# QizhiPei/FABind

Measured on AMD Instinct MI355X. Metric: complexes/sec fwd+bwd (1500p/40l nodes), full IaBNet on the whole graph (pocket model + 4-layer complex model + distance-map head on all nodes / pairs) with the pocket-cls + pocket-centre + coord + distmap + distmap-by-coords + distill losses (BASELINE configs[2] read literally), higher is better.
Workload: dtype bf16

## Files before the change

### fabind_amd/_lib.py

```python
import ctypes
import os

import torch

from . import config as _cfg

_HERE = os.path.dirname(os.path.abspath(__file__))
LIB_PATH = _cfg.knob("FABIND_LIB") or os.path.join(_HERE, "libfabind_hip.so")

ABI_VERSION = 19
DT_F32, DT_BF16 = 0, 1
ACT_NONE, ACT_SILU, ACT_RELU, ACT_SIGMOID, ACT_STORED_DERIV = 0, 1, 2, 3, 4
GEMM_FAM_NT_F32, GEMM_FAM_NT_F32_BF16, GEMM_FAM_NT_BF16, GEMM_FAM_GLDS, GEMM_FAM_PIPE, GEMM_FAM_X3, GEMM_FAM_X3_PRO, GEMM_FAM_PERSIST = range(8)

LNR_8S16, LNR_8S32, LNR_V8_1, LNR_V8_2, LNR_V8_3, LNR_V8_4, LNR_S2, LNR_S8, LNR_S16, LNR_S32, LNR_COUNT = range(11)
LNB_8S16, LNB_8S32, LNB_V8_1, LNB_V8_2, LNB_V8_3, LNB_S2, LNB_S8, LNB_S16, LNB_S20, LNB_S32, LNB_COUNT = range(11)
RST_BF16_1, RST_BF16_2, RST_BF16_4, RST_GENERIC, RST_COUNT = range(5)
ELF_WAVE1, ELF_WAVE1_TAIL, ELF_WAVE2_TAIL, ELF_CHUNK, ELF_COUNT = range(5)
ELB_NPL1, ELB_NPL2, ELB_NPL3, ELB_COUNT = range(4)

_vp, _i, _f, _l = ctypes.c_void_p, ctypes.c_int, ctypes.c_float, ctypes.c_long


class GemmArgs(ctypes.Structure):
# ... 125 lines not shown
    "fabind_rowdot_bwd": [_vp, _i, _vp, _i, _vp, _i, _i, _i, _vp, _vp, _vp, _i, _vp],
    "fabind_edge_geom_bwd": [_vp, _vp, _vp, _vp, _vp, _vp, _vp, _vp, _vp, _vp, _i, _i, _i, _vp, _vp, _vp, _vp],
    "fabind_gcl_pre_bwd": [_vp, _i, _i, _vp, _vp, _i, _vp, _vp, _vp, _i, _vp],
    "fabind_gather_dact": [_vp, _i, _vp, _vp, _i, _i, _vp, _i, _i, _i, _vp],
    "fabind_coord_update_bwd": [_vp, _vp, _vp, _i, _i, _f, _vp, _vp, _vp, _vp],
    "fabind_cross_attn_bwd": [_vp, _i, _vp, _i, _vp, _i, _i, _i, _vp, _i, _i, _i, _f, _vp, _vp, _vp, _vp, _vp, _vp, _vp,
                              _vp, _vp, _vp],
    "fabind_pair_bias_cat": [_vp, _i, _vp, _i, _i, _i, _vp, _i, _vp, _i, _vp, _vp, _i, _vp, _i, _vp, _vp],
    "fabind_batched_transpose_pad": [_vp, _i, _vp, _i, _i, _i, _i, _vp, _vp],
    "fabind_node_chain_fwd": [_vp, _i, _vp, _i, _vp, _vp, _vp, _vp, _vp, _vp, _i, _i, _vp, _i, _vp, _i, _vp, _i, _i, _i, _vp],
    "fabind_node_chain_x3_fwd": [_vp, _i, _vp, _i, _vp, _vp, _vp, _vp, _vp, _vp, _vp, _vp, _vp, _vp, _i, _i, _vp, _i, _vp, _i, _vp, _i, _vp, _i, _vp, _i,
                                 _i, _i, _vp],
    "fabind_rows_hadamard_bwd": [_vp, _i, _i, _vp, _i, _i, _vp, _vp, _vp, _i, _vp, _i, _vp],
    "fabind_pair_hadamard_bwd_grid": [_vp, _i, _i, _vp, _i, _i, _vp, _vp, _vp, _vp, _i, _vp, _i, _vp],
    "fabind_pair_hadamard_bwd_rows": [_vp, _i, _i, _vp, _i, _i, _vp, _i, _i, _vp, _vp, _vp, _vp, _i, _vp, _i, _vp, _i, _vp],
    "fabind_pair_hadamard_bwd": [_vp, _i, _i, _vp, _vp, _i, _i, _vp, _vp, _i, _i, _vp, _vp, _i, _vp, _vp, _i, _vp, _vp, _i,
                                 _vp],
    "fabind_inter_attn_bwd": [_vp, _i, _vp, _i, _i, _vp, _vp, _vp, _vp, _vp, _vp, _vp, _vp, _vp, _vp, _vp, _vp, _f, _i,
                              _vp, _vp, _vp, _vp, _vp, _vp, _vp, _vp, _vp, _vp, _i, _vp],
    "fabind_inter_attn_bwd_rows": [_vp, _i, _vp, _i, _i, _vp, _vp, _vp, _vp, _vp, _vp, _vp, _vp, _vp, _vp, _vp, _vp, _f, _i,
                                   _vp, _vp, _vp, _vp, _vp, _vp, _vp, _vp, _vp, _vp, _i, _vp, _i, _i, _vp],
    "fabind_las_step_bwd": [_vp, _vp, _vp, _vp, _vp, _vp, _vp, _vp, _i, _i, _f, _f, _vp, _vp, _vp],
    "fabind_pair_bias_bwd": [_vp, _i, _vp, _i, _i, _vp, _vp, _i, _i, _i, _vp, _vp, _vp, _vp, _vp],
    "fabind_pair_bias_btcat": [_vp, _i, _vp, _vp, _vp, _i, _i, _i, _vp, _i, _i, _vp],
    "fabind_pair_bias_finish": [_vp, _vp, _i, _i, _vp, _vp, _i, _vp, _vp, _l, _vp],
    "fabind_pack_frag_multi": [_vp, _vp, _i, _vp],
    "fabind_lower_bound": [_vp, _i, _vp, _i, _vp, _vp],
    "fabind_pocket_center_fwd": [_vp, _vp, _vp, _vp, _i, _i, _f, _i, _vp, _vp, _vp],
    "fabind_pocket_center_bwd": [_vp, _vp, _vp, _vp, _i, _i, _f, _vp, _vp, _vp, _vp, _vp],
    "fabind_pair_dist_fwd": [_vp, _i, _i, _vp, _vp, _f, _f, _f, _vp, _vp],
    "fabind_pair_dist_bwd": [_vp, _i, _i, _vp, _vp, _vp, _f, _f, _f, _vp, _vp, _vp],
    "fabind_block_hadamard_fwd": [_vp, _i, _i, _vp, _i, _vp, _i, _i, _vp, _i, _vp],
    "fabind_block_hadamard_bwd": [_vp, _i, _i, _vp, _i, _vp, _i, _vp, _i, _i, _vp, _i, _i, _vp, _vp, _i, _vp, _i, _vp],
    "fabind_loss_fwd": [_vp, _vp, _l, _vp, _vp, _vp, _l, _vp, _vp, _i, _vp, _l, _vp, _vp, _l, _f, _f, _f, _f, _f, _f, _vp, _vp, _vp, _vp, _vp, _vp],
    "fabind_loss_bwd": [_vp, _vp, _l, _vp, _vp, _vp, _l, _vp, _vp, _i, _l, _vp, _vp, _l, _f, _f, _f, _f, _f, _f, _vp, _vp, _vp,
                        _vp, _vp, _vp, _vp, _vp, _vp],
    "fabind_layernorm_fwd": [_vp, _vp, _vp, _f, _i, _i, _vp, _vp, _vp, _vp],
    "fabind_layernorm_bwd": [_vp, _vp, _vp, _vp, _vp, _i, _i, _vp, _vp, _vp, _vp],
}

_lib = None


def load():
    global _lib
    if _lib is not None:
        return _lib
    if not os.path.exists(LIB_PATH):
        raise RuntimeError(
            "fabind_amd: %s is missing -- build it with `python -m fabind_amd.build` (hipcc, gfx950). "
            "There is no CPU/eager fallback for the hot path." % LIB_PATH)
    lib = ctypes.CDLL(LIB_PATH)
    lib.fabind_last_error.restype = ctypes.c_char_p
    lib.fabind_abi_version.restype = ctypes.c_int
    got = lib.fabind_abi_version()
    if got != ABI_VERSION:
        raise RuntimeError("fabind_amd: %s has ABI version %d, this binding needs %d -- rebuild with `python -m fabind_amd.build`"
                           % (LIB_PATH, got, ABI_VERSION))
    lib.fabind_sizeof_args.argtypes, lib.fabind_sizeof_args.restype = [ctypes.c_int], ctypes.c_int
    lib.fabind_cross_attn_bwd_scratch.argtypes, lib.fabind_cross_attn_bwd_scratch.restype = [_i, _i, _i], ctypes.c_long
    lib.fabind_pair_bias_cat_parts.argtypes, lib.fabind_pair_bias_cat_parts.restype = [_i, _i], ctypes.c_long
    lib.fabind_cross_attn_fused_bwd_scratch.argtypes, lib.fabind_cross_attn_fused_bwd_scratch.restype = [_i, _i, _i, _i, _i], ctypes.c_long
    lib.fabind_cross_attn_fused_bwd_parts.argtypes, lib.fabind_cross_attn_fused_bwd_parts.restype = [_i, _i], ctypes.c_int
    lib.fabind_pair_bias_finish_parts.argtypes, lib.fabind_pair_bias_finish_parts.restype = [_i], ctypes.c_int
    lib.fabind_loss_blocks.argtypes, lib.fabind_loss_blocks.restype = [_l, _l, _l], ctypes.c_int
    for nm in ("fabind_pair_block_tile", "fabind_pair_block_chunk"):
# ... 58 lines not shown
```

### fabind_amd/build.py

```python
import os
import subprocess
import sys

HERE = os.path.dirname(os.path.abspath(__file__))
CSRC = os.path.join(HERE, "csrc")
INCLUDE = os.path.join(os.path.dirname(HERE), "include")
LIB = os.path.join(HERE, "libfabind_hip.so")
SOURCES = ["capi.hip", "gemm.hip", "graph.hip", "gcl.hip", "fused_edge.hip", "fused_edge_fwd2.hip", "fused_edge_fwd3.hip", "fused_edge_bwd3.hip", "fused_edge_bwd4.hip", "pair_fused.hip", "attn.hip", "inter_attn_rows.hip", "attn_mfma.hip", "norm.hip", "bwd.hip", "post_optim.hip", "distgen.hip", "node_chain.hip", "heads.hip", "symmetry.hip", "pose_cluster.hip", "optim.hip", "ranking.hip", "conformer.hip", "topology.hip"]
HIPCC = os.environ.get("HIPCC", "/opt/rocm/bin/hipcc")
FLAGS = ["--offload-arch=gfx950", "-O3", "-std=c++17", "-fPIC", "-Wno-comment", "-I" + INCLUDE, "-I" + CSRC]


def _stale(out, deps):
    if not os.path.exists(out):
        return True
    t = os.path.getmtime(out)
    return any(os.path.getmtime(d) > t for d in deps)


def build(force=False, verbose=True):
    objs = []
    hdrs = [os.path.join(CSRC, "common.h"), os.path.join(CSRC, "fused_common.h"), os.path.join(INCLUDE, "fabind_hip.h")]
    procs = []
    for src in SOURCES:
        sp = os.path.join(CSRC, src)
        if not os.path.exists(sp):
            raise RuntimeError("fabind_amd.build: source %s is missing" % sp)
        obj = os.path.join(CSRC, src.replace(".hip", ".o"))
        objs.append(obj)
        if force or _stale(obj, [sp] + hdrs):
            cmd = [HIPCC] + FLAGS + ["-c", sp, "-o", obj]
            if verbose:
                print(" ".join(cmd), flush=True)
            procs.append((src, subprocess.Popen(cmd)))
    for src, p in procs:
        if p.wait() != 0:
            raise RuntimeError("hipcc failed on " + src)
    if force or procs or _stale(LIB, objs):
        cmd = [HIPCC, "--offload-arch=gfx950", "-shared", "-fPIC", "-o", LIB] + objs
        if verbose:
            print(" ".join(cmd), flush=True)
# ... 7 lines not shown
```

### fabind_amd/kernels.py

```python
import ctypes

import numpy as np
import torch

from . import _lib
from . import config as _cfg
from ._lib import ACT_NONE, ACT_RELU, ACT_SIGMOID, ACT_SILU, ACT_STORED_DERIV, GemmArgs, check, dt_code, ptr, stream

__all__ = ["gemm", "colsum", "edges_count", "edges_fill", "exclusive_scan", "inter_meta",
           "edge_geom", "gcl_pre", "segment_sum", "coord_update", "cross_attn_fwd", "pair_bmat", "pair_hadamard",
           "inter_attn_fwd", "las_step", "select_rows", "ACT_NONE", "ACT_SILU", "ACT_RELU", "ACT_SIGMOID", "ACT_STORED_DERIV"]

GEMM_BN = 128
GEMM_DEFAULT_CONFIG = 13
PROFILE = None
PROFILE_ONLY = None


PROFILE_BYTES = {}
PROFILE_ALGO = {}


def _profiled(label, flops, fn, nbytes=0.0, algo=None):
    if PROFILE is None or (PROFILE_ONLY is not None and not label.startswith(PROFILE_ONLY)):
# ... 992 lines not shown
                                      dy.numel(), float(scale), stream()), "fabind_mul_dact")
    return out


def mul_dact_colsum(dy, aux, act, out_dtype, scale=1.0):
    R, C = dy.shape
    out = torch.empty((R, C), dtype=out_dtype, device=dy.device)
    nchunk = _nchunk_fused(R)
    scratch = torch.empty((nchunk, C), dtype=torch.float32, device=dy.device)
    db = torch.empty(C, dtype=torch.float32, device=dy.device)
    check(_lib.load().fabind_mul_dact_colsum(ptr(dy), dt_code(dy.dtype), ptr(aux), dt_code(aux.dtype) if aux is not None else 0,
                                             act, ptr(out), dt_code(out_dtype), R, C, ptr(db), ptr(scratch), nchunk, float(scale),
                                             stream()), "fabind_mul_dact_colsum")
    return out, db


def mul_dropmask_colsum(dy, p_drop, seed, out_dtype):
    R, C = dy.shape
    out = torch.empty((R, C), dtype=out_dtype, device=dy.device)
    nchunk = _nchunk_fused(R)
    scratch = torch.empty((nchunk, C), dtype=torch.float32, device=dy.device)
    db = torch.empty(C, dtype=torch.float32, device=dy.device)
    check(_lib.load().fabind_mul_dropmask_colsum(ptr(dy), dt_code(dy.dtype), ptr(out), dt_code(out_dtype), R, C, float(p_drop),
                                                 int(seed) & 0xFFFFFFFF, ptr(db), ptr(scratch), nchunk, stream()),
          "fabind_mul_dropmask_colsum")
    return out, db


def rowdot_bwd(z, dpart, u, act_epi):
    M, N = z.shape
    dz = torch.empty_like(z)
    nchunk = _nchunk(M)
    scratch = torch.empty((nchunk, N), dtype=torch.float32, device=z.device)
    du = torch.empty(N, dtype=torch.float32, device=z.device)
    check(_lib.load().fabind_rowdot_bwd(ptr(z), dt_code(z.dtype), ptr(dpart), dpart.shape[1], ptr(u), act_epi, M, N,
                                        ptr(dz), ptr(du), ptr(scratch), nchunk, stream()), "fabind_rowdot_bwd")
    return dz, du


def edge_geom_bwd(d, rho, norm, dd, drhohat, row, rowptr, colptr, perm, node_off, B, n):
    E, dev = row.shape[0], d.device
    dx = torch.empty((n, 3), dtype=torch.float32, device=dev)
    gbuf, gnorm = torch.empty((max(E, 1), 3), dtype=torch.float32, device=dev), torch.empty(B, dtype=torch.float32, device=dev)
    check(_lib.load().fabind_edge_geom_bwd(ptr(d), ptr(rho), ptr(norm), ptr(dd), ptr(drhohat), ptr(row), ptr(rowptr), ptr(colptr),
                                           ptr(perm), ptr(node_off), B, E, n, ptr(dx), ptr(gbuf), ptr(gnorm), stream()),
          "fabind_edge_geom_bwd")
    return dx


def gcl_pre_bwd(dpre, H, rhohat, w_r):
    E = dpre.shape[0]
    drh = torch.empty(E, dtype=torch.float32, device=dpre.device)
    nchunk = max(1, min(2048, (E + 255) // 256))
    scratch = torch.empty((nchunk, H), dtype=torch.float32, device=dpre.device)
    dw = torch.empty(H, dtype=torch.float32, device=dpre.device)
    check(_lib.load().fabind_gcl_pre_bwd(ptr(dpre), dt_code(dpre.dtype), H, ptr(rhohat), ptr(w_r), E, ptr(drh), ptr(dw),
                                         ptr(scratch), nchunk, stream()), "fabind_gcl_pre_bwd")
    return drh, dw


def gather_dact(dout, row, Z, act):
    dZ = torch.empty_like(Z)
    check(_lib.load().fabind_gather_dact(ptr(dout), _ld(dout), ptr(row), ptr(Z), dt_code(Z.dtype), act, ptr(dZ),
                                         dt_code(dZ.dtype), Z.shape[0], Z.shape[1], stream()), "fabind_gather_dact")
    return dZ


# ... 49 lines not shown
    check(_lib.load().fabind_pair_hadamard_bwd_grid(ptr(dhd), dt_code(dhd.dtype), _ld(dhd), ptr(T), _ld(T), Hh, ptr(node_off), ptr(c_cnt),
                                                    ptr(node_b), ptr(desc_p), N, ptr(dT), _ld(dT), stream()),
          "fabind_pair_hadamard_bwd_grid")


def rows_hadamard_bwd(dout, t, rowptr, pair_idx, partner):
    dt_ = torch.empty_like(t)
    check(_lib.load().fabind_rows_hadamard_bwd(ptr(dout), dt_code(dout.dtype), _ld(dout), ptr(t), _ld(t), t.shape[1], ptr(rowptr),
                                               ptr(pair_idx), ptr(partner), t.shape[0], ptr(dt_), _ld(dt_), stream()),
          "fabind_rows_hadamard_bwd")
    return dt_


def pair_block_tile_chunk():
    return _lib.load().fabind_pair_block_tile(), _lib.load().fabind_pair_block_chunk()


def block_hadamard_fwd(bl, t, n_a):
    W = t.shape[1]
    out = torch.empty((bl.n_pairs, W), dtype=torch.bfloat16, device=t.device)
    check(_lib.load().fabind_block_hadamard_fwd(bl.desc_ptr, bl.B, bl.n_tiles, ptr(t), _ld(t), ptr(t[n_a:]), _ld(t), W, ptr(out), W,
                                                stream()), "fabind_block_hadamard_fwd")
    return out


def block_hadamard_bwd(bl, dout, t, n_a):
    W = t.shape[1]
    dt_ = torch.empty_like(t)
    part = torch.empty((bl.n_tiles, bl.nchunk_max, bl.chunk, W), dtype=torch.float32, device=t.device)
    check(_lib.load().fabind_block_hadamard_bwd(bl.desc_ptr, bl.B, bl.n_tiles, ptr(dout), _ld(dout), ptr(t), _ld(t), ptr(t[n_a:]), _ld(t),
                                                W, bl.row_b_ptr, bl.n_crows, bl.nchunk_max, ptr(part), ptr(dt_), _ld(dt_),
                                                ptr(dt_[n_a:]), _ld(dt_), stream()), "fabind_block_hadamard_bwd")
    return dt_


def inter_attn_bwd(qkv, cv, H, d, rhohat, rowptr, col, mirror, red_idx, w_rk, w_rv, wcr, w3, alpha, cvs, clampv, dh_out, dx_out, nblk,
                   deal=None):
    N, E = qkv.shape[0], col.shape[0]
    f32 = dict(dtype=torch.float32, device=qkv.device)
    dqkv = torch.empty_like(qkv)
    dcv = torch.empty_like(cv)
    dd, drh = torch.empty((max(E, 1), 3), **f32), torch.empty(max(E, 1), **f32)
    n_red = E // 2
    dbias_red = torch.zeros(max(n_red, 1), **f32)
    dlogit, dcp = torch.empty(max(E, 1), **f32), torch.empty(max(E, 1), **f32)
    if E == 0:
        dd.zero_(); drh.zero_()
    wpart = torch.empty((nblk, 4 * H), **f32)
    args = (ptr(qkv), _ld(qkv), ptr(cv), _ld(cv), H, ptr(d), ptr(rhohat), ptr(rowptr), ptr(col), ptr(mirror), ptr(red_idx), ptr(w_rk),
            ptr(w_rv), ptr(wcr), ptr(w3), ptr(alpha), ptr(cvs), clampv, N, ptr(dh_out), ptr(dx_out), ptr(dqkv), ptr(dcv), ptr(dd), ptr(drh),
            ptr(dbias_red), ptr(dlogit), ptr(dcp), ptr(wpart), nblk)
    if deal is not None:
        check(_lib.load().fabind_inter_attn_bwd_rows(*args, ptr(deal[0]), int(deal[1]), int(deal[2]), stream()), "fabind_inter_attn_bwd_rows")
    else:
        check(_lib.load().fabind_inter_attn_bwd(*args, stream()), "fabind_inter_attn_bwd")
    return dqkv, dcv, dd[:E], drh[:E], dbias_red[:n_red], dcp[:E], colsum(wpart)


def las_step_bwd(x, x0, mask, las_i, las_j, las_off, node_off, c_cnt, B, max_n, step, clampv, dout):
    dx = torch.empty_like(x)
    check(_lib.load().fabind_las_step_bwd(ptr(x), ptr(x0), ptr(mask), ptr(las_i), ptr(las_j), ptr(las_off), ptr(node_off), ptr(c_cnt), B,
                                          max_n, step, clampv, ptr(dout), ptr(dx), stream()), "fabind_las_step_bwd")
    return dx


def pair_bias_cat(douts, lay, H, Kp, b0, wcomp):
# ... 188 lines not shown
```

### fabind_amd/models/model.py

```python
import random

import torch
import torch.nn as nn
import torch.nn.functional as F
from torch.nn import Linear

from .. import kernels as K
from .. import ops
from ..utils.utils import get_keepNode_tensor, gumbel_softmax_no_random
from .att_model import EfficientMCAttModel


class Transition_diff_out_dim(nn.Module):

    def __init__(self, embedding_channels=256, out_channels=256, n=4):
        super().__init__()
        self.layernorm = nn.LayerNorm(embedding_channels)
        self.linear1 = Linear(embedding_channels, n * embedding_channels)
        self.linear2 = Linear(n * embedding_channels, out_channels)
        torch.nn.init.xavier_uniform_(self.linear1.weight, gain=0.001)
        torch.nn.init.xavier_uniform_(self.linear2.weight, gain=0.001)

    def forward(self, z):
        shp = z.shape
# ... 252 lines not shown
        start = _offsets(reps)
        j = torch.arange(pi.shape[0], device=dev) - start[pi]
        ci = _offsets(ncnt)[pocket_batch][pi] + j
        kn = torch.stack([kcnt, ncnt]).tolist()
        return _Pairs(pi, ci, ops.PairBlocks(kn[0], kn[1], dev))

    def _complex_and_heads(self, data, g, plan=None):
        scale = self.coordinate_scale
        cb = data['compound'].batch
        if plan:
            Xn, Xl, cidx, pidx = plan['Xn'], plan['Xl'], plan['cidx'], plan['pidx']
        else:
            Xn = self.normalize_coord(g['X'].unsqueeze(-2)).float()
            Xl = self.normalize_coord(g['XL'].unsqueeze(-2)).float()
            seg1 = g['segment'].bool() if not g['segment'].is_floating_point() else g['segment'] > 0.5
            cidx = torch.nonzero(~seg1 & ~g['is_global']).squeeze(1)
            pidx = torch.nonzero(seg1 & ~g['is_global']).squeeze(1)
        Xo, Ho = self.complex_model(Xn, g['H'], batch_id=g['batch'], segment_id=g['segment'], mask=g['mask'],
                                    is_global=g['is_global'], compound_edge_index=g['c2c'], LAS_edge_index=g['LAS'],
                                    batched_complex_coord_LAS=Xl, LAS_mask=None)
        coords_n = ops.take_unique_rows(Xo, cidx).squeeze(-2)
        return Ho, cidx, pidx, coords_n

    def _dist_heads(self, data, g, Ho, cidx, pidx, coords_n):
        cb = data['compound'].batch
        pairs = g.get('pairs')
        if pairs is None:
            B = int(cb[-1].item()) + 1
            pairs = self._pair_lists(g['pocket_batch'], cb, torch.bincount(g['pocket_batch'], minlength=B), torch.bincount(cb, minlength=B))
        pi, ci = pairs
        ln = ops.layernorm(ops.take_unique_rows(Ho, torch.cat([pidx, cidx])), self.layernorm.weight, self.layernorm.bias, self.layernorm.eps)
        npk = pidx.shape[0]
        blocks = getattr(pairs, 'blocks', None)
        hd = ops.rows_hadamard(ln, pi, npk + ci, a_sorted=True, blocks=blocks, n_a=npk)
        wd = ops.mm_dtype()
        part = ops.linear_rowdot(hd, self.distmap_mlp[0].weight.to(wd), self.distmap_mlp[0].bias,
                                 self.distmap_mlp[2].weight[0].contiguous(), act_epi=K.ACT_RELU)
        y_pred = (part.sum(1) + self.distmap_mlp[2].bias).sigmoid() * 10
        xp = self.normalize_coord(g['pocket_xyz']).float()
        if blocks is not None and coords_n.is_cuda:
            y_by = ops.pair_dist(xp, coords_n, blocks, scale=self.coordinate_scale, lo=0.0, hi=10.0)
        else:
            y_by = self.unnormalize_coord((xp[pi] - ops.take_rows_few(coords_n, ci)).norm(dim=-1)).clamp(0, 10)
        return y_pred, y_by

    def forward(self, data, stage=1, train=False, plan=None):
        cb = data['compound'].batch
        if plan is not None:
            self._adopt_plan(plan, cb.device)
        if plan is not None:
            keep_idx = plan['keep_idx']
        else:
            keep_idx = torch.nonzero(data['pocket'].keepNode).squeeze(1) if (stage == 1 or self.pocket_pred_model.training) else None
        head = self._pocket_head(data, plan)
        training = self.pocket_pred_model.training
        center = self._soft_center(head['logits'], head['mask'], head['xyz'], noise=training)
        pocket_cls = torch.zeros_like(head['mask'], dtype=data.pocket_idx.dtype)
        pocket_cls[head['pb'], head['loc']] = data.pocket_idx
        if training:
            dist = torch.norm(data.coords_center - center, p=2, dim=-1).mean(dim=-1)
            final_stage = 2 if (dist < self.args.center_dist_threshold and random.random() < self.stage_prob) else 1
        else:
            final_stage = stage
        if final_stage == 2:
            c2 = center
            if self.args.local_eval or (self.args.train_pred_pocket_noise and train):
                c2 = center + self.args.train_pred_pocket_noise * (2 * torch.rand_like(center) - 1)
            g = self._stage2(data, head, c2)
        else:
            cx = data['complex']
            pemb = ops.take_unique_rows(head['p_out'], keep_idx if keep_idx is not None else torch.nonzero(data['pocket'].keepNode).squeeze(1))
# ... 62 lines not shown
```

### fabind_amd/ops.py

```python
import numpy as np
import torch

from . import config as _cfg
from . import kernels as K


def act_dtype():
    return torch.float32 if _cfg.fp32_storage() else torch.bfloat16


mm_dtype = act_dtype


def needs_grad(*ts):
    return torch.is_grad_enabled() and any(torch.is_tensor(t) and t.requires_grad for t in ts)


_needs_grad = needs_grad


def _ksplit(R):
    S = max(1, min(128, R // 4096))
    unit = 64 * S
    return S, (R + unit - 1) // unit * unit
# ... 1528 lines not shown
    m8 = p_mask.contiguous().view(torch.uint8) if p_mask.dtype == torch.bool else p_mask.to(torch.uint8).contiguous()
    w = {k: float(v) for k, v in w.items()}
    loss, terms = _SixTermLoss.apply(f(coords), f(y_pred), f(y_by), f(logits), f(center), f(coords_true), f(dis_map), cls, m8,
                                     f(center_true), w)
    tt = terms.unbind(0)
    return loss, {n: tt[i] for i, n in enumerate(LOSS_TERM_NAMES)}


_PAIRBLOCK = np.dtype([("pair_off", np.int64), ("P", np.int32), ("C", np.int32), ("p_row0", np.int32), ("c_row0", np.int32),
                       ("tile0", np.int32), ("pad", np.int32)])


class PairBlocks:

    def __init__(self, kcnt, ncnt, dev):
        from .param_pack import _upload
        kc, nc = np.asarray(kcnt, dtype=np.int64), np.asarray(ncnt, dtype=np.int64)
        B = kc.shape[0]
        tp, ch = K.pair_block_tile_chunk()
        tiles = (kc + tp - 1) // tp
        d = np.zeros(B, dtype=_PAIRBLOCK)
        d["pair_off"] = np.cumsum(kc * nc) - kc * nc
        d["P"], d["C"] = kc, nc
        d["p_row0"], d["c_row0"] = np.cumsum(kc) - kc, np.cumsum(nc) - nc
        d["tile0"] = np.cumsum(tiles) - tiles
        self.B, self.n_tiles, self.n_pairs = int(B), int(tiles.sum()), int((kc * nc).sum())
        self.max_C, self.n_prows, self.n_crows = int(nc.max()) if B else 0, int(kc.sum()), int(nc.sum())
        self.nchunk_max = (self.max_C + ch - 1) // ch
        self.chunk = ch
        row_b = np.repeat(np.arange(B, dtype=np.int32), nc)
        raw = np.concatenate([d.view(np.uint8), row_b.view(np.uint8)]) if B else np.zeros(0, dtype=np.uint8)
        self.buf = _upload(raw, dev) if raw.shape[0] else None
        self.desc_bytes = d.view(np.uint8).shape[0]

    def tensors(self):
        return [self.buf] if self.buf is not None else []

    @property
    def desc_ptr(self):
        return self.buf.data_ptr()

    @property
    def row_b_ptr(self):
        return self.buf.data_ptr() + self.desc_bytes


class _PairDist(torch.autograd.Function):
    @staticmethod
    def forward(ctx, xp, xc, blocks, scale, lo, hi):
        ctx.save_for_backward(xp, xc)
        ctx.blocks, ctx.k = blocks, (scale, lo, hi)
        return K.pair_dist_fwd(blocks, xp, xc, scale, lo, hi)

    @staticmethod
    def backward(ctx, dy):
        xp, xc = ctx.saved_tensors
        return None, K.pair_dist_bwd(ctx.blocks, xp, xc, dy.contiguous().float(), ctx.k[0], ctx.k[1], ctx.k[2]), None, None, None, None


def pair_dist(xp, xc, blocks, scale=1.0, lo=0.0, hi=10.0):
    assert not xp.requires_grad, "pair_dist: the pocket coordinates are data"
    xp, xc = xp.float().contiguous(), xc.float().contiguous()
    assert xp.shape[0] == blocks.n_prows and xc.shape[0] == blocks.n_crows
    return _PairDist.apply(xp, xc, blocks, float(scale), float(lo), float(hi))


RANK_MODES = {"logsigmoid": 0, "dynamic_hinge": 1}
RANK_MAX_GROUP = 1024
COUNT_NAMES = ("ranked_right", "pairs", "hit", "confidence_correct")


def atom_offsets(compound_batch, B):
    cb = compound_batch.to(torch.int32).contiguous()
    return K.lower_bound(cb, torch.arange(B + 1, dtype=torch.int32, device=cb.device), B + 1)


def pose_stats(pred, truth, compound_batch, B):
    if pred.dim() != 2 or pred.shape[1] != 3 or tuple(truth.shape) != tuple(pred.shape):
        raise ValueError("pose_stats: pred and truth must both be [N, 3]; got %s and %s" % (tuple(pred.shape), tuple(truth.shape)))
    if compound_batch.dim() != 1 or compound_batch.numel() != pred.shape[0]:
        raise ValueError("pose_stats: compound_batch must be [N = %d]; got %s" % (pred.shape[0], tuple(compound_batch.shape)))
    if B < 0 or pred.shape[0] >= 2 ** 31 // 3:
        raise ValueError("pose_stats: B >= 0 and fewer than 2^31 / 3 atoms")
    p, t = pred.detach().float().contiguous(), truth.detach().float().contiguous()
    return K.pose_stats(p, t, atom_offsets(compound_batch, B), B)


class _RankLoss(torch.autograd.Function):
    @staticmethod
    def forward(ctx, scores, rmsd, group_off, G, mode, with_ce):
        terms, d_scores, counts = K.rank_loss_fwd(scores, rmsd, group_off, G, mode, with_ce)
        mean = terms.mean(0)
        ranking, ce, loss = mean.unbind(0)
        ctx.save_for_backward(d_scores)
        ctx.G = G
        ctx.mark_non_differentiable(ranking, ce, terms, counts)
        return loss, ranking, ce, terms, counts
# ... 34 lines not shown
```

### include/fabind_hip.h

```cpp
#ifndef FABIND_HIP_H
#define FABIND_HIP_H

#include <stdint.h>

#ifdef __cplusplus
extern "C" {
#endif

#ifndef __HIP_PLATFORM_AMD__
typedef struct ihipStream_t* hipStream_t;
#endif

const char* fabind_last_error(void);
#define FABIND_ABI_VERSION 19
int fabind_abi_version(void);
int fabind_sizeof_args(int which);

typedef struct FabindGemmArgs {
    const void* A;
    const void* A2;
    const void* W;
    void* C;
    const float* bias;
    const void* R;
// ... 263 lines not shown
int fabind_las_step(const float* x, const float* x0, const int* las_i, const int* las_j, const int* las_off,
                    const int* node_off, const int* c_cnt, int B, int max_n, float step, float clampv, float* x_out,
                    unsigned char* pass_mask, hipStream_t stream);

int fabind_pocket_center_fwd(const float* logits, const uint8_t* mask, const float* xyz, const float* noise, int B, int L,
                             float tau, int hard, float* center, float* wsum, hipStream_t stream);
int fabind_pocket_center_bwd(const float* logits, const uint8_t* mask, const float* xyz, const float* noise, int B, int L,
                             float tau, const float* center, const float* wsum, const float* dcenter, float* dlogits,
                             hipStream_t stream);

int fabind_loss_blocks(long n_pair, long n_coord, long n_cls);
int fabind_loss_fwd(const float* coords, const float* coords_true, long n_coord, const float* y_pred, const float* y_by,
                    const float* dis_map, long n_pair, const float* logits, const void* cls, int cls_dt, const uint8_t* mask,
                    long n_cls, const float* center, const float* center_true, long n_center, float w_coord, float w_pair,
                    float w_distill, float w_cls, float w_center, float delta, float* part, unsigned* ticket, float* out,
                    float* loss_out, float* terms_out, hipStream_t stream);
int fabind_loss_bwd(const float* coords, const float* coords_true, long n_coord, const float* y_pred, const float* y_by,
                    const float* dis_map, long n_pair, const float* logits, const void* cls, int cls_dt, long n_cls,
                    const float* center, const float* center_true, long n_center, float w_coord, float w_pair, float w_distill,
                    float w_cls, float w_center, float delta, const float* fwd_out, const float* g_loss, const float* g_terms,
                    float* d_coords, float* d_y_pred, float* d_y_by, float* d_logits, float* d_center, hipStream_t stream);

int fabind_pair_block_tile(void);
int fabind_pair_block_chunk(void);
int fabind_pair_dist_fwd(const void* desc, int B, int n_tiles, const float* xp, const float* xc, float scale, float lo, float hi,
                         float* y, hipStream_t stream);
int fabind_pair_dist_bwd(const void* desc, int B, int max_C, const float* xp, const float* xc, const float* dy, float scale, float lo,
                         float hi, float* part, float* dxc, hipStream_t stream);
int fabind_block_hadamard_fwd(const void* desc, int B, int n_tiles, const float* tp, int ldtp, const float* tc, int ldtc, int W, void* out,
                              int ldo, hipStream_t stream);
int fabind_block_hadamard_bwd(const void* desc, int B, int n_tiles, const void* dout, int ldo, const float* tp, int ldtp,
                              const float* tc, int ldtc, int W, const int* row_b, int n_crows, int nchunk_max, float* part,
                              float* dtp, int lddp, float* dtc, int lddc, hipStream_t stream);

int fabind_select_rows(const float* x, const float* z, const uint8_t* mask, int n, int width, float* x_out,
                       hipStream_t stream);

int fabind_row_stats(const void* x, int x_dt, int ldx, float eps, int R, int C, float* mu, float* rs, hipStream_t stream);

int fabind_layernorm_rows(const void* x, int x_dt, int ldx, const float* w, const float* b, float eps, int R, int C, void* y,
                          int y_dt, int ldy, int pad_to, hipStream_t stream);
int fabind_edge_ln_concat(const float* h, int ldh, int H, const int* row, const int* col, const float* rhohat, const float* w,
                          const float* b, float eps, int E, void* y, int y_dt, int ldy, int pad_to, hipStream_t stream);

int fabind_edge_lnfold(const void* AB, int ldab, int Kp, int H, const int* row, const int* col, const float* rho,
                       const float* stat, float eps, const float* w_r, const float* c_r, const float* c_c, const float* dvec,
                       int E, void* out, float p_drop, unsigned seed, hipStream_t stream);
int fabind_edge_lnfold_bwd_blocks(int E);
int fabind_edge_lnfold_bwd(const void* AB, int ldab, int Kp, int H, const int* row, const int* col, const float* rho,
                           const float* stat, float eps, const float* w_r, const float* c_r, const float* c_c,
                           const void* out, const void* dout, int E, float p_drop, void* du, float* es,
                           float* drho, float* part, int n_blocks, hipStream_t stream);

int fabind_inter_coord_fold(const void* P, int ldp, int H, const int* col, const float* rho, const float* stat, float q_w,
                            float eps, const float* u, const float* d, const float* w3, int E, float* s_out, float p_drop,
                            unsigned seed, hipStream_t stream);
int fabind_layernorm_rows_bwd(const void* x, int x_dt, int ldx, const float* w, const void* dy, int dy_dt, int lddy, float eps,
                              int R, int C, void* dx, int dx_dt, int lddx, float* dw_part, float* db_part, int nblk, hipStream_t stream);
int fabind_edge_concat(const float* h, int ldh, int H, const int* row, const int* col, const float* rhohat, int E, void* y,
                       int y_dt, int ldy, int pad_to, hipStream_t stream);
int fabind_layernorm_fwd(const float* x, const float* w, const float* b, float eps, int R, int C, float* y, float* mean,
                         float* rstd, hipStream_t stream);
int fabind_layernorm_bwd(const float* x, const float* w, const float* dy, const float* mean, const float* rstd, int R,
                         int C, float* dx, float* dw_part, float* db_part, hipStream_t stream);

#define FB_LNR_8S16 0
// ... 137 lines not shown
```

Measured before the change: 539.2.

## Fuse distance-map head hadamard, linear, relu and rowdot into one kernel

Adds a HIP kernel that builds the pocket×compound hadamard rows in LDS per block, runs the 512×512 first distmap linear via MFMA, and reduces relu(z)·u in place. This replaces separate rows_hadamard and linear_rowdot launches and avoids rereading the hadamard tensor from memory. In training it still stores z and hd for backward, so the write traffic stays. Compute runs serially over compound columns per block, so parallelism depends on the tile count.

```diff
diff --git a/fabind_amd/_lib.py b/fabind_amd/_lib.py
--- a/fabind_amd/_lib.py
+++ b/fabind_amd/_lib.py
@@ -181,6 +181,7 @@
     "fabind_pair_dist_bwd": [_vp, _i, _i, _vp, _vp, _vp, _f, _f, _f, _vp, _vp, _vp],
     "fabind_block_hadamard_fwd": [_vp, _i, _i, _vp, _i, _vp, _i, _i, _vp, _i, _vp],
     "fabind_block_hadamard_bwd": [_vp, _i, _i, _vp, _i, _vp, _i, _vp, _i, _i, _vp, _i, _i, _vp, _vp, _i, _vp, _i, _vp],
+    "fabind_dist_head_fwd": [_vp, _i, _i, _vp, _vp, _i, _i, _vp, _vp, _vp, _l, _vp, _vp, _vp, _vp],
     "fabind_loss_fwd": [_vp, _vp, _l, _vp, _vp, _vp, _l, _vp, _vp, _i, _vp, _l, _vp, _vp, _l, _f, _f, _f, _f, _f, _f, _vp, _vp, _vp, _vp, _vp, _vp],
     "fabind_loss_bwd": [_vp, _vp, _l, _vp, _vp, _vp, _l, _vp, _vp, _i, _l, _vp, _vp, _l, _f, _f, _f, _f, _f, _f, _vp, _vp, _vp,
                         _vp, _vp, _vp, _vp, _vp, _vp],
diff --git a/fabind_amd/build.py b/fabind_amd/build.py
--- a/fabind_amd/build.py
+++ b/fabind_amd/build.py
@@ -6,7 +6,7 @@
 CSRC = os.path.join(HERE, "csrc")
 INCLUDE = os.path.join(os.path.dirname(HERE), "include")
 LIB = os.path.join(HERE, "libfabind_hip.so")
-SOURCES = ["capi.hip", "gemm.hip", "graph.hip", "gcl.hip", "fused_edge.hip", "fused_edge_fwd2.hip", "fused_edge_fwd3.hip", "fused_edge_bwd3.hip", "fused_edge_bwd4.hip", "pair_fused.hip", "attn.hip", "inter_attn_rows.hip", "attn_mfma.hip", "norm.hip", "bwd.hip", "post_optim.hip", "distgen.hip", "node_chain.hip", "heads.hip", "symmetry.hip", "pose_cluster.hip", "optim.hip", "ranking.hip", "conformer.hip", "topology.hip"]
+SOURCES = ["capi.hip", "gemm.hip", "graph.hip", "gcl.hip", "fused_edge.hip", "fused_edge_fwd2.hip", "fused_edge_fwd3.hip", "fused_edge_bwd3.hip", "fused_edge_bwd4.hip", "pair_fused.hip", "attn.hip", "inter_attn_rows.hip", "attn_mfma.hip", "norm.hip", "bwd.hip", "post_optim.hip", "distgen.hip", "node_chain.hip", "heads.hip", "dist_head.hip", "symmetry.hip", "pose_cluster.hip", "optim.hip", "ranking.hip", "conformer.hip", "topology.hip"]
 HIPCC = os.environ.get("HIPCC", "/opt/rocm/bin/hipcc")
 FLAGS = ["--offload-arch=gfx950", "-O3", "-std=c++17", "-fPIC", "-Wno-comment", "-I" + INCLUDE, "-I" + CSRC]
 
diff --git a/fabind_amd/csrc/dist_head.hip b/fabind_amd/csrc/dist_head.hip
--- /dev/null
+++ b/fabind_amd/csrc/dist_head.hip
@@ -0,0 +1,147 @@
+#include "common.h"
+#include "fabind_hip.h"
+#include "fused_common.h"
+
+namespace {
+
+constexpr int DH_H = 512;
+constexpr int DH_TP = 128;
+constexpr int DH_SWZ = 15;
+
+struct PairBlock { long pair_off; int P, C, p_row0, c_row0, tile0, pad; };
+
+__device__ __forceinline__ int dh_find(const PairBlock* __restrict__ desc, int B, int tile) {
+    int lo = 0, hi = B - 1;
+    while (lo < hi) {
+        const int mid = (lo + hi + 1) >> 1;
+        if (desc[mid].tile0 <= tile) lo = mid; else hi = mid - 1;
+    }
+    return lo;
+}
+
+typedef __attribute__((ext_vector_type(4))) unsigned int dh_u4;
+
+__device__ __forceinline__ int dh_fresh(int lane) {
+    asm volatile("" : "+v"(lane));
+    return lane;
+}
+
+template <bool STORE>
+__global__ __launch_bounds__(DH_H, 4) void dist_head_fwd_kernel(const PairBlock* __restrict__ desc, int B, const float* __restrict__ tp,
+                                                                const float* __restrict__ tc, int ldt, const bf16_t* __restrict__ W1p,
+                                                                const float* __restrict__ b1, const float* __restrict__ u, long n_pairs,
+                                                                float* y_lin, bf16_t* z, bf16_t* hd) {
+    constexpr int H = DH_H;
+    extern __shared__ __attribute__((aligned(16))) unsigned char smem[];
+    bf16_t* sX = (bf16_t*)smem;
+    float* sDot = (float*)(sX + FE_BM * H);
+    const int tid = threadIdx.x, lane = tid & 63, wave = __builtin_amdgcn_readfirstlane(tid >> 6);
+    const int dtile = blockIdx.x >> 1;
+    const PairBlock d = desc[dh_find(desc, B, dtile)];
+    const int i0 = (dtile - d.tile0) * DH_TP + (blockIdx.x & 1) * FE_BM;
+    if (i0 >= d.P || d.C <= 0) return;
+    const int np = min(FE_BM, d.P - i0);
+
+    for (int ja = 0; ja < d.C; ++ja) {
+        {
+            const int l8 = dh_fresh(lane) * 8;
+            const float* cr = tc + (size_t)(d.c_row0 + ja) * ldt + l8;
+            const float4 c0 = *(const float4*)cr, c1 = *(const float4*)(cr + 4);
+            float4 p0[FE_BM / 8], p1[FE_BM / 8];
+#pragma unroll
+            for (int k = 0; k < FE_BM / 8; ++k) {
+                const float* pr = tp + (size_t)(d.p_row0 + i0 + min(wave + 8 * k, np - 1)) * ldt + l8;
+                p0[k] = *(const float4*)pr;
+                p1[k] = *(const float4*)(pr + 4);
+            }
+#pragma unroll
+            for (int k = 0; k < FE_BM / 8; ++k) {
+                const int rw = wave + 8 * k;
+                uint4 v = make_uint4(pack2_bf16(p0[k].x * c0.x, p0[k].y * c0.y), pack2_bf16(p0[k].z * c0.z, p0[k].w * c0.w),
+                                     pack2_bf16(p1[k].x * c1.x, p1[k].y * c1.y), pack2_bf16(p1[k].z * c1.z, p1[k].w * c1.w));
+                if (rw >= np) v = make_uint4(0u, 0u, 0u, 0u);
+                if (STORE) {
+                    const long row = d.pair_off + (long)(i0 + rw) * d.C + ja;
+                    if (rw < np && row < n_pairs) __builtin_nontemporal_store(dh_u4{v.x, v.y, v.z, v.w}, (dh_u4*)(hd + (size_t)row * H + l8));
+                }
+                *(uint4*)&sX[rw * H + (l8 ^ ((rw & DH_SWZ) * 8))] = v;
+            }
+        }
+        __syncthreads();
+        f32x4_t acc[4][4];
+        fe_zero(acc);
+        fe_gemm_rolled<H, 4, false, DH_SWZ>(sX, W1p, wave, lane, acc);
+        if (STORE) __syncthreads();
+        const int le = dh_fresh(lane), fr = le & 15, cq = le >> 4;
+        float bj[4], uj[4];
+#pragma unroll
+        for (int j = 0; j < 4; ++j) { bj[j] = b1[wave * 64 + j * 16 + fr]; uj[j] = u[wave * 64 + j * 16 + fr]; }
+#pragma unroll
+        for (int i = 0; i < 4; ++i) {
+            float ds[4] = {0.f, 0.f, 0.f, 0.f};
+#pragma unroll
+            for (int j = 0; j < 4; ++j) {
+                const int colj = wave * 64 + j * 16 + fr;
+#pragma unroll
+                for (int r = 0; r < 4; ++r) {
+                    const int rw = i * 16 + cq * 4 + r;
+                    const float vp = acc[i][j][r] + bj[j];
+                    if (STORE) sX[rw * H + (((colj >> 3) ^ (rw & DH_SWZ)) * 8) + (colj & 7)] = f32_to_bf16(vp);
+                    ds[r] += fmaxf(vp, 0.f) * uj[j];
+                }
+            }
+#pragma unroll
+            for (int r = 0; r < 4; ++r) {
+                float t = ds[r];
+                t += __shfl_xor(t, 1, 64); t += __shfl_xor(t, 2, 64); t += __shfl_xor(t, 4, 64); t += __shfl_xor(t, 8, 64);
+                if (fr == 0) sDot[wave * FE_BM + i * 16 + cq * 4 + r] = t;
+            }
+        }
+        __syncthreads();
+        if (STORE) {
+            const int l8 = dh_fresh(lane) * 8;
+#pragma unroll
+            for (int k = 0; k < FE_BM / 8; ++k) {
+                const int rw = wave + 8 * k;
+                const long row = d.pair_off + (long)(i0 + rw) * d.C + ja;
+                if (rw < np && row < n_pairs) {
+                    const uint4 v = *(const uint4*)&sX[rw * H + (l8 ^ ((rw & DH_SWZ) * 8))];
+                    __builtin_nontemporal_store(dh_u4{v.x, v.y, v.z, v.w}, (dh_u4*)(z + (size_t)row * H + l8));
+                }
+            }
+        }
+        if (tid < np) {
+            float t = 0.f;
+#pragma unroll
+            for (int w = 0; w < H / 64; ++w) t += sDot[w * FE_BM + tid];
+            const long row = d.pair_off + (long)(i0 + tid) * d.C + ja;
+            if (row < n_pairs) y_lin[row] = t;
+        }
+    }
+}
+
+}
+
+extern "C" int fabind_dist_head_fwd(const void* desc, int B, int n_tiles, const float* tp, const float* tc, int ldt, int W, const void* W1p,
+                                    const float* b1, const float* u, long n_pairs, float* y_lin, void* z, void* hd, hipStream_t stream) {
+    FB_REQUIRE(W == DH_H, "fabind_dist_head_fwd: W must be 512");
+    FB_REQUIRE(ldt % 4 == 0 && ((((uintptr_t)tp | (uintptr_t)tc | (uintptr_t)W1p | (uintptr_t)z | (uintptr_t)hd) & 15) == 0),
+               "fabind_dist_head_fwd: 16-byte aligned rows");
+    FB_REQUIRE((z == nullptr) == (hd == nullptr), "fabind_dist_head_fwd: z and hd are stored together or not at all");
+    FB_REQUIRE(fabind_pair_block_tile() == DH_TP, "fabind_dist_head_fwd: descriptor tiles of 128 residues");
+    if (B <= 0 || n_tiles <= 0 || n_pairs <= 0) return 0;
+    FB_REQUIRE(W1p && b1 && u && y_lin, "fabind_dist_head_fwd: W1p, b1, u and y_lin are required");
+    const dim3 grid(2 * (unsigned)n_tiles);
+    const size_t lds = (size_t)FE_BM * DH_H * 2 + (size_t)(DH_H / 64) * FE_BM * sizeof(float);
+#define DH_LAUNCH(ST)                                                                                                              \
+    do {                                                                                                                           \
+        static bool set_ = false;                                                                                                  \
+        if (!set_) { (void)hipFuncSetAttribute((const void*)dist_head_fwd_kernel<ST>, hipFuncAttributeMaxDynamicSharedMemorySize, (int)lds); set_ = true; } \
+        hipLaunchKernelGGL((dist_head_fwd_kernel<ST>), grid, dim3(DH_H), lds, stream, (const PairBlock*)desc, B, tp, tc, ldt,      \
+                           (const bf16_t*)W1p, b1, u, n_pairs, y_lin, (bf16_t*)z, (bf16_t*)hd);                                    \
+    } while (0)
+    if (z != nullptr) DH_LAUNCH(true); else DH_LAUNCH(false);
+#undef DH_LAUNCH
+    FB_CHECK_LAUNCH();
+    return 0;
+}
diff --git a/fabind_amd/kernels.py b/fabind_amd/kernels.py
--- a/fabind_amd/kernels.py
+++ b/fabind_amd/kernels.py
@@ -1048,7 +1048,7 @@
     dz = torch.empty_like(z)
     nchunk = _nchunk(M)
     scratch = torch.empty((nchunk, N), dtype=torch.float32, device=z.device)
-    du = torch.empty(N, dtype=torch.float32, device=z.device)
+    du = (torch.empty if M else torch.zeros)(N, dtype=torch.float32, device=z.device)
     check(_lib.load().fabind_rowdot_bwd(ptr(z), dt_code(z.dtype), ptr(dpart), dpart.shape[1], ptr(u), act_epi, M, N,
                                         ptr(dz), ptr(du), ptr(scratch), nchunk, stream()), "fabind_rowdot_bwd")
     return dz, du
@@ -1164,6 +1164,19 @@
                                                 W, bl.row_b_ptr, bl.n_crows, bl.nchunk_max, ptr(part), ptr(dt_), _ld(dt_),
                                                 ptr(dt_[n_a:]), _ld(dt_), stream()), "fabind_block_hadamard_bwd")
     return dt_
+
+
+def dist_head_fused_fwd(bl, t, n_a, W1p, b1, u, store):
+    W = t.shape[1]
+    n = bl.n_pairs
+    y = torch.empty((n,), dtype=torch.float32, device=t.device)
+    z = torch.empty((n, W), dtype=torch.bfloat16, device=t.device) if store else None
+    hd = torch.empty((n, W), dtype=torch.bfloat16, device=t.device) if store else None
+    _profiled("dist_head_fused_fwd pairs=%d%s" % (n, " (z, hd stored)" if store else ""), 2.0 * n * W * W,
+              lambda: check(_lib.load().fabind_dist_head_fwd(bl.desc_ptr, bl.B, bl.n_tiles, ptr(t), ptr(t[n_a:]), _ld(t), W, ptr(W1p), ptr(b1),
+                                                             ptr(u), n, ptr(y), ptr(z), ptr(hd), stream()), "fabind_dist_head_fwd"),
+              4.0 * n + 2.0 * W * W + 4.0 * t.shape[0] * W + (4.0 * n * W if store else 0.0))
+    return y, z, hd
 
 
 def inter_attn_bwd(qkv, cv, H, d, rhohat, rowptr, col, mirror, red_idx, w_rk, w_rv, wcr, w3, alpha, cvs, clampv, dh_out, dx_out, nblk,
diff --git a/fabind_amd/models/model.py b/fabind_amd/models/model.py
--- a/fabind_amd/models/model.py
+++ b/fabind_amd/models/model.py
@@ -308,11 +308,9 @@
         ln = ops.layernorm(ops.take_unique_rows(Ho, torch.cat([pidx, cidx])), self.layernorm.weight, self.layernorm.bias, self.layernorm.eps)
         npk = pidx.shape[0]
         blocks = getattr(pairs, 'blocks', None)
-        hd = ops.rows_hadamard(ln, pi, npk + ci, a_sorted=True, blocks=blocks, n_a=npk)
-        wd = ops.mm_dtype()
-        part = ops.linear_rowdot(hd, self.distmap_mlp[0].weight.to(wd), self.distmap_mlp[0].bias,
-                                 self.distmap_mlp[2].weight[0].contiguous(), act_epi=K.ACT_RELU)
-        y_pred = (part.sum(1) + self.distmap_mlp[2].bias).sigmoid() * 10
+        y_lin = ops.dist_head(ln, blocks, npk, self.distmap_mlp[0].weight.to(ops.mm_dtype()), self.distmap_mlp[0].bias,
+                              self.distmap_mlp[2].weight[0].contiguous(), idx_a=pi, idx_b=npk + ci)
+        y_pred = (y_lin + self.distmap_mlp[2].bias).sigmoid() * 10
         xp = self.normalize_coord(g['pocket_xyz']).float()
         if blocks is not None and coords_n.is_cuda:
             y_by = ops.pair_dist(xp, coords_n, blocks, scale=self.coordinate_scale, lo=0.0, hi=10.0)
diff --git a/fabind_amd/ops.py b/fabind_amd/ops.py
--- a/fabind_amd/ops.py
+++ b/fabind_amd/ops.py
@@ -1584,6 +1584,15 @@
         raw = np.concatenate([d.view(np.uint8), row_b.view(np.uint8)]) if B else np.zeros(0, dtype=np.uint8)
         self.buf = _upload(raw, dev) if raw.shape[0] else None
         self.desc_bytes = d.view(np.uint8).shape[0]
+        self._counts = (kc, nc)
+
+    def pair_lists(self, dev):
+        kc, nc = self._counts
+        pi = np.repeat(np.arange(int(kc.sum()), dtype=np.int64), np.repeat(nc, kc))
+        c0 = np.repeat(np.cumsum(nc) - nc, kc * nc)
+        j = np.arange(pi.shape[0], dtype=np.int64) - np.repeat(np.cumsum(kc * nc) - kc * nc, kc * nc)
+        ci = c0 + (j % np.maximum(np.repeat(nc, kc * nc), 1))
+        return (torch.from_numpy(pi.astype(np.int32)).to(dev), torch.from_numpy(ci.astype(np.int32)).to(dev))
 
     def tensors(self):
         return [self.buf] if self.buf is not None else []
@@ -1615,6 +1624,49 @@
     xp, xc = xp.float().contiguous(), xc.float().contiguous()
     assert xp.shape[0] == blocks.n_prows and xc.shape[0] == blocks.n_crows
     return _PairDist.apply(xp, xc, blocks, float(scale), float(lo), float(hi))
+
+
+DIST_HEAD_FUSED = True
+
+
+class _DistHead(torch.autograd.Function):
+    @staticmethod
+    def forward(ctx, t, W1, b1, u, blocks, n_a):
+        y, z, hd = K.dist_head_fused_fwd(blocks, t, n_a, K.pack_frag(W1), b1, u, store=True)
+        ctx.blocks, ctx.n_a, ctx.Wt = blocks, n_a, _stored_wt(W1)
+        ctx.save_for_backward(t, W1, u, z, hd)
+        return y
+
+    @staticmethod
+    def backward(ctx, g):
+        t, W1, u, z, hd = ctx.saved_tensors
+        if z.shape[0] == 0:
+            return torch.zeros_like(t), torch.zeros_like(W1), torch.zeros_like(u), torch.zeros_like(u), None, None
+        dpart = g.float().unsqueeze(1).expand(-1, (W1.shape[0] + K.GEMM_BN - 1) // K.GEMM_BN).contiguous()
+        dz, du = _rowdot_bwd(z, dpart, u, K.ACT_RELU)
+        dhd, _ = K.gemm(dz, _wt(ctx.Wt, W1), out_dtype=hd.dtype)
+        dW, db = _param_grads(dz, hd, None, W1, True, True)
+        return K.block_hadamard_bwd(ctx.blocks, dhd, t, ctx.n_a), dW, db, du, None, None
+
+
+def _dist_head_fits(t, blocks, n_a, W1):
+    return (DIST_HEAD_FUSED and act_dtype() == torch.bfloat16 and t.is_cuda and t.dtype == torch.float32 and t.dim() == 2 and t.is_contiguous()
+            and t.shape[1] == 512 and blocks is not None and n_a == blocks.n_prows and t.shape[0] == blocks.n_prows + blocks.n_crows
+            and tuple(W1.shape) == (512, 512) and W1.dtype == torch.bfloat16)
+
+
+def dist_head(t, blocks, n_a, W1, b1, u, idx_a=None, idx_b=None):
+    if _dist_head_fits(t, blocks, n_a, W1):
+        b1, u = b1.float().contiguous(), u.float().contiguous()
+        if _needs_grad(t, W1, b1, u):
+            K.tn_hook(W1, b1)
+            return _DistHead.apply(t, W1.contiguous(), b1, u, blocks, n_a)
+        return K.dist_head_fused_fwd(blocks, t, n_a, K.pack_frag(W1), b1, u, store=False)[0]
+    if idx_a is None:
+        idx_a, idx_b = blocks.pair_lists(t.device)
+        idx_b = n_a + idx_b
+    hd = rows_hadamard(t, idx_a, idx_b, a_sorted=True, blocks=blocks, n_a=n_a)
+    return linear_rowdot(hd, W1, b1, u, act_epi=K.ACT_RELU).sum(1)
 
 
 RANK_MODES = {"logsigmoid": 0, "dynamic_hinge": 1}
diff --git a/include/fabind_hip.h b/include/fabind_hip.h
--- a/include/fabind_hip.h
+++ b/include/fabind_hip.h
@@ -319,6 +319,8 @@
 int fabind_block_hadamard_bwd(const void* desc, int B, int n_tiles, const void* dout, int ldo, const float* tp, int ldtp,
                               const float* tc, int ldtc, int W, const int* row_b, int n_crows, int nchunk_max, float* part,
                               float* dtp, int lddp, float* dtc, int lddc, hipStream_t stream);
+int fabind_dist_head_fwd(const void* desc, int B, int n_tiles, const float* tp, const float* tc, int ldt, int W, const void* W1p,
+                         const float* b1, const float* u, long n_pairs, float* y_lin, void* z, void* hd, hipStream_t stream);
 
 int fabind_select_rows(const float* x, const float* z, const uint8_t* mask, int n, int width, float* x_out,
                        hipStream_t stream);
```

Measured after the change: 534.1. About the same (-0.9%).
